# ProgramerSalar/stable-diffusion-from-scratch

Measured on NVIDIA B200. Metric: 512px DDIM-50 images/sec, higher is better.
Workload: dtype bf16

## Files before the change

include/sdb200.h:

```cpp
#ifndef SDB200_H
#define SDB200_H

#include <stdint.h>

#ifdef __cplusplus
extern "C" {
#endif

#define SDB_OK            0
#define SDB_ERR_INVALID  -1
#define SDB_ERR_CUDA     -2
#define SDB_ERR_NOTMA    -3

#define SDB_F32   0
#define SDB_BF16  1

int         sdb_version(void);
const char* sdb_last_error_string(void);
int         sdb_device_sm_count(void);
unsigned long long sdb_launch_count(void);
int sdb_pdl_skip_next(int n);

int sdb_nchw_to_nhwc(const float* src, void* dst, int dst_dtype, int N, int C, int dst_C, int HW, void* stream);
int sdb_nchw_to_nhwc_split(const float* src, void* dst , int N, int C, int dst_C, int HW, void* stream);
// ... 83 lines not shown
    int geglu;
    int col_group, col_group_stride;
    int split_k;
    int block_n;
    int taps;
    int kw;
    int stride, pad_h, pad_w;
    int NB, IH, IW, Cin, OH, OW;
    int cout_pad;
    int out_sh, out_sw, out_oh, out_ow, OHF, OWF;
    void* ws; long long ws_bytes;
    int rows_per_item;
    int variant;
    float* colstats; long long colstats_slots;
    int b_const;
} sdb_tc_args;
int sdb_tc_colstats_layout(const sdb_tc_args* args , long long* slots, long long* slots_per_item);
long long sdb_tc_workspace_bytes(const sdb_tc_args* args );
int sdb_tc_contract(const sdb_tc_args* args , void* stream);
int sdb_tc_set_pair_kernel(int enable);
int sdb_tc_set_tma_epilogue(int enable);
int sdb_tc_set_tail_split(int enable);

typedef struct sdb_attn_args {
    const void* q; const void* k; const void* v; void* out;
    long long q_bs, q_ss, q_hs;
    long long k_bs, k_ss, k_hs;
    long long v_bs, v_ss, v_hs;
    long long o_bs, o_ss, o_hs;
    int B, H, Sq, Sk, d, dpad;
    float scale;
    int dense;
    int causal;
// ... 13 lines not shown
```

stable-diffusion-from-scratch_b200/_lib.py:

```python
import ctypes as C
import os

import torch

HERE = os.path.dirname(os.path.abspath(__file__))
LIB_PATH = os.path.join(HERE, "libsdb200.so")

F32, BF16 = 0, 1

_lib = None


class SdbError(RuntimeError):
    pass


class SimtArgs(C.Structure):
    _fields_ = [
        ("A", C.c_void_p), ("B", C.c_void_p), ("out", C.c_void_p),
        ("bias", C.c_void_p), ("rowvec", C.c_void_p), ("residual", C.c_void_p),
        ("lda", C.c_longlong), ("ldb", C.c_longlong), ("ldc", C.c_longlong), ("ldr", C.c_longlong), ("ldv", C.c_longlong),
        ("M", C.c_int), ("N", C.c_int), ("K", C.c_int),
        ("alpha", C.c_float),
        ("b_kn", C.c_int),
# ... 15 lines not shown
        ("out_dtype", C.c_int),
        ("geglu", C.c_int),
        ("col_group", C.c_int), ("col_group_stride", C.c_int),
        ("split_k", C.c_int),
        ("block_n", C.c_int),
        ("taps", C.c_int), ("kw", C.c_int),
        ("stride", C.c_int), ("pad_h", C.c_int), ("pad_w", C.c_int),
        ("NB", C.c_int), ("IH", C.c_int), ("IW", C.c_int), ("Cin", C.c_int), ("OH", C.c_int), ("OW", C.c_int),
        ("cout_pad", C.c_int),
        ("out_sh", C.c_int), ("out_sw", C.c_int), ("out_oh", C.c_int), ("out_ow", C.c_int), ("OHF", C.c_int), ("OWF", C.c_int),
        ("ws", C.c_void_p), ("ws_bytes", C.c_longlong),
        ("rows_per_item", C.c_int),
        ("variant", C.c_int),
        ("colstats", C.c_void_p), ("colstats_slots", C.c_longlong),
        ("b_const", C.c_int),
    ]


class AttnArgs(C.Structure):
    _fields_ = [
        ("q", C.c_void_p), ("k", C.c_void_p), ("v", C.c_void_p), ("out", C.c_void_p),
        ("q_bs", C.c_longlong), ("q_ss", C.c_longlong), ("q_hs", C.c_longlong),
        ("k_bs", C.c_longlong), ("k_ss", C.c_longlong), ("k_hs", C.c_longlong),
        ("v_bs", C.c_longlong), ("v_ss", C.c_longlong), ("v_hs", C.c_longlong),
        ("o_bs", C.c_longlong), ("o_ss", C.c_longlong), ("o_hs", C.c_longlong),
        ("B", C.c_int), ("H", C.c_int), ("Sq", C.c_int), ("Sk", C.c_int), ("d", C.c_int), ("dpad", C.c_int),
        ("scale", C.c_float),
        ("dense", C.c_int),
        ("causal", C.c_int),
    ]
# ... 29 lines not shown
    "sdb_gather_rows": (_I, [_P, _P, _I, _I, _P, _P]),
    "sdb_skinny_linear": (_I, [_P, _I, _I, _P, _P, _I, _I, _I, _P, _P]),
    "sdb_skinny_linear_bf16w": (_I, [_P, _I, _I, _P, _P, _I, _I, _I, _P, _P]),
    "sdb_ddim_step": (_I, [_P, _P, _P, _F, _P, _F, _F, _F, _F, _F, _F, _P, _P, _L, _P]),
    "sdb_ddim_xprev": (_I, [_P, _P, _P, _F, _P, _F, _F, _F, _F, _P, _L, _P]),
    "sdb_ddpm_step": (_I, [_P, _P, _P, _P, _P, _P, _I, _I, _F, _P, _P, _I, _L, _P]),
    "sdb_inpaint_blend": (_I, [_P, _P, _P, _P, _P, _P, _I, _I, _I, _L, _P, _P]),
    "sdb_diag_gaussian": (_I, [_P, _P, _I, _I, _L, _P, _P, _P, _P, _P, _P]),
    "sdb_q_sample": (_I, [_P, _P, _P, _P, _I, _L, _P, _P]),
    "sdb_simt_contract": (_I, [C.POINTER(SimtArgs), _P]),
    "sdb_tc_contract": (_I, [C.POINTER(TcArgs), _P]),
    "sdb_tc_set_pair_kernel": (_I, [_I]),
    "sdb_tc_set_tma_epilogue": (_I, [_I]),
    "sdb_tc_set_tail_split": (_I, [_I]),
    "sdb_tc_workspace_bytes": (_L, [C.POINTER(TcArgs)]),
    "sdb_tc_colstats_layout": (_I, [C.POINTER(TcArgs), C.POINTER(C.c_longlong), C.POINTER(C.c_longlong)]),
    "sdb_attention_fwd": (_I, [C.POINTER(AttnArgs), _P]),
    "sdb_attention_set_short_key_kernel": (_I, [_I]),
    "sdb_attention_wide_fwd": (_I, [_P, _P, _P, _P, _L, _L, _L, _L, _L, _L, _L, _L, _I, _I, _I, _I, _F, _P]),
}


def load(path=None):
    global _lib
    if _lib is not None and path is None:
        return _lib
    path = path or LIB_PATH
    if not os.path.exists(path):
        raise SdbError(
            "libsdb200.so not found at %s — build it with `python -c 'import __graft_entry__ as g; g.build()'`; "
# ... 51 lines not shown
```

stable-diffusion-from-scratch_b200/csrc/tc_contract.cu:

```cuda
#include "common.cuh"
#include "ptx.cuh"
#include <stdlib.h>
#include <string.h>

namespace sdb {

using namespace ptx;

struct TcP {
    void* out;
    const float* bias; const float* rowvec; const float* residual;
    float* ws; long long ws_split_stride;
    float* colstats; long long colstats_sq;
    long long ldc, ldr, ldv;
    int M, N;
    int kblocks;
    int kpt;
    int out_bf16, geglu;
    int col_group, col_group_stride;
    int split_k;
    int tiles_n;
    int m_pairs;
    int off32;
    int stages;
    int epi_tma;
    int epi_nbuf;
    int epi_bw, epi_bh;
// ... 444 lines not shown
        for (int o = 8; o <= 16; o <<= 1) {
            cs_s.x += __shfl_xor_sync(0xffffffffu, cs_s.x, o); cs_s.y += __shfl_xor_sync(0xffffffffu, cs_s.y, o);
            cs_s.z += __shfl_xor_sync(0xffffffffu, cs_s.z, o); cs_s.w += __shfl_xor_sync(0xffffffffu, cs_s.w, o);
            cs_q.x += __shfl_xor_sync(0xffffffffu, cs_q.x, o); cs_q.y += __shfl_xor_sync(0xffffffffu, cs_q.y, o);
            cs_q.z += __shfl_xor_sync(0xffffffffu, cs_q.z, o); cs_q.w += __shfl_xor_sync(0xffffffffu, cs_q.w, o);
        }
        const int cn = col + 4 * (int)qd;
        if (lane < 8 && cn < n_out) {
            float* dst = p.colstats + (long long)(ub.mt * 4 + lg) * p.N + cn;
            *reinterpret_cast<float4*>(dst) = cs_s;
            *reinterpret_cast<float4*>(dst + p.colstats_sq) = cs_q;
        }
    }
}

template <int BN, int MODE, bool HAS_RES>
__device__ __forceinline__ void epilogue_tma_units(const TcP& p, const CUtensorMap* tmC, const CUtensorMap* tmR, uint32_t tmem_d,
                                                   float* s_bias2, uint32_t stg_a, uint64_t* rbar, uint64_t* tfull_bar,
                                                   uint32_t tempty_leader0, uint32_t tempty_leader1, int warp, int lane, uint32_t rank,
                                                   int pair, int npairs, int units) {
    constexpr bool GEGLU = MODE == EPI_GEGLU;
    constexpr bool OUT16 = MODE != EPI_F32;
    constexpr int COLS = GEGLU ? BN / 2 : BN;
    constexpr int NCHUNK = (COLS + 31) / 32;
    constexpr int CPW_MAX = (NCHUNK + 1) / 2;
    constexpr int ACC_STRIDE = 256;
    const int lg = warp & 3, half = (warp - 4) >> 2;
    const int et = threadIdx.x - 128;
    const int cpw = (NCHUNK - half + 1) / 2;
    const int nbuf = p.epi_nbuf, lead = nbuf - 1;
    const bool partial = p.split_k > 1;
    const float* const biasp = partial ? nullptr : p.bias;
    const float* const rowv = (!partial && p.rowvec && p.conv && MODE == EPI_F32) ? p.rowvec : nullptr;
    const bool want_cs = MODE == EPI_F32 && p.colstats != nullptr && !partial;
    const int n_out = GEGLU ? p.N / 2 : p.N;
// ... 98 lines not shown
                if (lane == 0) mbar_arrive_cluster(buf ? tempty_leader1 : tempty_leader0);
            }
            if (HAS_RES) {
                mbar_wait(rbar + bi, (q / (uint32_t)nbuf) & 1u);
            } else {
                if (lane == 0) tma_store_wait_read<1>();
                __syncwarp();
            }
            tepi_chunk<BN, MODE, HAS_RES>(p, tmC, cur, g, sb_a, sbuf, c0, col, ub, lane, lg, rowmask, img_w, rv_ok, rowv, want_cs, partial, n_out);
            if (HAS_RES) {
                if (lane == 0) tma_store_wait_read<1>();
                issue_residual(q + (uint32_t)lead);
            }
            ++q;
        }
    }
    if (lane == 0) tma_store_wait_read<0>();
    __syncwarp();
}

template <int BN, int MODE, bool HAS_RES>
__device__ __forceinline__ void epilogue_tma_single(const TcP& p, const CUtensorMap* tmC, const CUtensorMap* tmR, uint32_t taddr,
                                                    uint32_t sb_a, uint32_t stg_a, uint64_t* rbar, uint64_t* accum_bar, const UnitBox& ub,
                                                    int lane, int lg, uint32_t rowmask, int img_w, int ncols) {
    constexpr bool GEGLU = MODE == EPI_GEGLU;
    constexpr int COLS = GEGLU ? BN / 2 : BN;
    constexpr int NCHUNK = (COLS + 31) / 32;
    const int nch = ncols >= COLS ? NCHUNK : (ncols + 31) / 32;
    const bool partial = p.split_k > 1;
    const float* const rowv = (!partial && p.rowvec && p.conv && MODE == EPI_F32) ? p.rowvec : nullptr;
// ... 38 lines not shown
tc_contract_kernel(const __grid_constant__ CUtensorMap tmA, const __grid_constant__ CUtensorMap tmB,
                   const __grid_constant__ CUtensorMap tmC, const __grid_constant__ CUtensorMap tmR, const TcP p) {
    pdl_trigger();
    if (threadIdx.x == 0) { TC1_TRACE(0); TC1_TRACE(7); }
    using Cfg = TcCfg<BN>;
    constexpr int STAGES = Cfg::STAGES;
    extern __shared__ uint8_t smem_raw[];
    uint8_t* smem = reinterpret_cast<uint8_t*>((reinterpret_cast<uintptr_t>(smem_raw) + 1023) & ~(uintptr_t)1023);
    uint8_t* sA = smem;
    uint8_t* sB = smem + STAGES * TC_A_BYTES;
    uint64_t* full_bar = reinterpret_cast<uint64_t*>(smem + STAGES * Cfg::STAGE_BYTES);
    uint64_t* empty_bar = full_bar + STAGES;
    uint64_t* accum_bar = empty_bar + STAGES;
    uint32_t* tmem_slot = reinterpret_cast<uint32_t*>(accum_bar + 1);
    uint64_t* res_bar = accum_bar + 2;
    float* s_bias = reinterpret_cast<float*>(smem + STAGES * Cfg::STAGE_BYTES + 256);

    const int warp = threadIdx.x >> 5, lane = threadIdx.x & 31;

    int tile = blockIdx.x;
    int ncols = BN, n_off = 0;
    if (tile >= p.full_tiles) {
        const int t2 = tile - p.full_tiles;
        tile = p.full_tiles + (t2 >> 1);
        if (t2 & 1) { n_off = 96; ncols = BN - 96; } else { ncols = 96; }
    }
    const int nt = tile % p.tiles_n, mt = tile / p.tiles_n;
    const int n0 = nt * BN + n_off;
    const int split = blockIdx.y;
    const int kb0 = (int)((long long)p.kblocks * split / p.split_k);
// ... 119 lines not shown
#define SDB_TEPI1(MODE, RES) epilogue_tma_single<BN, MODE, RES>(p, &tmC, &tmR, taddr, smem_u32(s_bias), stg_a, rbar, accum_bar, ub, lane, lg, rowmask, img_w, ncols)
            if (p.geglu) {
                if constexpr (BN % 64 == 0) SDB_TEPI1(EPI_GEGLU, false);
            } else if (p.split_k > 1) SDB_TEPI1(EPI_F32, false);
            else if (p.out_bf16) SDB_TEPI1(EPI_BF16, false);
            else if (p.residual != nullptr) SDB_TEPI1(EPI_F32, true);
            else SDB_TEPI1(EPI_F32, false);
#undef SDB_TEPI1
        } else {
            prefetch_residual_row(p, pix, n0, BN);
            float* stage = reinterpret_cast<float*>(sA) + (warp - 2) * (EPI_WARP_BYTES / 4);
            if (warp == 2 && lane == 0) TC1_TRACE(4);
            epilogue_warp<BN>(p, taddr, s_bias, stage, lane, n0, nt, pix, img, split, 0, 1, accum_bar, 0, mt * 4 + lg, ncols);
            if (warp == 2 && lane == 0) TC1_TRACE(5);
        }
    }

    tcgen05_fence_before();
    __syncthreads();
    if (warp == 1) {
        tcgen05_fence_after();
        tmem_dealloc(tmem_d, Cfg::TMEM_COLS);
    }
}

constexpr int TC2_MAX_STAGES = 8;
constexpr int TC2_SMEM_LIMIT = 232448;

template <int BN, int EW>
struct Tc2Cfg {
// ... 16 lines not shown
                        const __grid_constant__ CUtensorMap tmC, const __grid_constant__ CUtensorMap tmR, const TcP p) {
    pdl_trigger();
    using Cfg = Tc2Cfg<BN, EW>;
    constexpr int TC2_EPI_WARPS = EW;
    const int STAGES = p.stages;
    extern __shared__ uint8_t smem_raw[];
    uint8_t* smem = reinterpret_cast<uint8_t*>((reinterpret_cast<uintptr_t>(smem_raw) + 1023) & ~(uintptr_t)1023);
    uint8_t* sA = smem;
    uint8_t* sB = smem + STAGES * TC_A_BYTES;
    uint64_t* full_bar = reinterpret_cast<uint64_t*>(smem + STAGES * Cfg::STAGE_BYTES);
    uint64_t* empty_bar = full_bar + TC2_MAX_STAGES;
    uint64_t* tfull_bar = empty_bar + TC2_MAX_STAGES;
    uint64_t* tempty_bar = tfull_bar + 2;
    uint32_t* tmem_slot = reinterpret_cast<uint32_t*>(tempty_bar + 2);
    uint64_t* res_bar = tempty_bar + 4;
    float* s_bias = reinterpret_cast<float*>(smem + STAGES * Cfg::STAGE_BYTES + 512);
    uint8_t* staging = reinterpret_cast<uint8_t*>((reinterpret_cast<uintptr_t>(s_bias + 2 * BN) + 1023) & ~(uintptr_t)1023);

    const int warp = threadIdx.x >> 5, lane = threadIdx.x & 31;
    const uint32_t rank = cluster_ctarank();
    const int pair = blockIdx.x >> 1, npairs = gridDim.x >> 1;
    const int units = p.m_pairs * p.tiles_n * p.split_k;

    if (warp == 0 && lane == 0) {
        tma_prefetch_desc(&tmA);
        tma_prefetch_desc(&tmB);
        for (int s = 0; s < STAGES; ++s) { mbar_init(&full_bar[s], 1); mbar_init(&empty_bar[s], 1); }
        for (int b = 0; b < 2; ++b) { mbar_init(&tfull_bar[b], 1); mbar_init(&tempty_bar[b], 2 * TC2_EPI_WARPS); }
        for (int b = 0; b < 3 * EW && EW == 8; ++b) mbar_init(&res_bar[b], 1);
        fence_barrier_init();
// ... 71 lines not shown
                    const uint64_t bdesc = bdesc0 + (uint64_t)(s * (Cfg::B_HALF_BYTES >> 4));
#pragma unroll
                    for (int k = 0; k < TC_BK / 16; ++k)
                        umma_bf16_ss_pair(acc, adesc + 2 * k, bdesc + 2 * k, idesc, (kb > kb0 || k > 0) ? 1u : 0u);
                    umma_commit_pair(&empty_bar[s], 3);
                    if (++s == STAGES) { s = 0; ph ^= 1; }
                }
                umma_commit_pair(&tfull_bar[buf], 3);
                TC_TRACE(2, it);
            }
        }
    } else if (warp >= 4 && EW == 8 && p.epi_tma) {
        const uint32_t tl0 = mapa_u32(&tempty_bar[0], 0), tl1 = mapa_u32(&tempty_bar[1], 0);
        const uint32_t stg_a = smem_u32(staging) + (uint32_t)(warp - 4) * (uint32_t)(p.epi_nbuf * TEPI_BOX_BYTES);
        uint64_t* rbar = res_bar + 3 * (warp - 4);
#define SDB_TEPI(MODE, RES) epilogue_tma_units<BN, MODE, RES>(p, &tmC, &tmR, tmem_d, s_bias, stg_a, rbar, tfull_bar, tl0, tl1, warp, lane, rank, pair, npairs, units)
        if (p.geglu) {
            if constexpr (BN % 64 == 0) SDB_TEPI(EPI_GEGLU, false);
        } else if (p.split_k > 1) SDB_TEPI(EPI_F32, false);
        else if (p.out_bf16) SDB_TEPI(EPI_BF16, false);
        else if (p.residual != nullptr) SDB_TEPI(EPI_F32, true);
        else SDB_TEPI(EPI_F32, false);
#undef SDB_TEPI
    } else if (warp >= 4) {
        const int et = threadIdx.x - 128;
        const int lg = warp & 3;
        const int half = (warp - 4) >> 2;
        const int row = lg * 32 + lane;
        const uint32_t tempty_leader0 = mapa_u32(&tempty_bar[0], 0);
        const uint32_t tempty_leader1 = mapa_u32(&tempty_bar[1], 0);
        float* stage = reinterpret_cast<float*>(staging) + (warp - 4) * (EPI_WARP_BYTES / 4);
        auto row_of = [&](int mt, int& img) -> long long {
            img = 0;
            if (p.conv) {
// ... 29 lines not shown
            for (int i = et; i < BN; i += 32 * TC2_EPI_WARPS) {
                int n = n0 + i;
                s_bias[i] = (p.bias && n < p.N) ? p.bias[n] : 0.f;
            }
            named_bar_sync(1, 32 * TC2_EPI_WARPS);
            int img = 0;
            const long long pix = row_of(mt, img);
            const uint32_t taddr = tmem_d + ((uint32_t)(lg * 32) << 16) + buf * Cfg::ACC_STRIDE;
            if (warp == 4 && lane == 0) TC_TRACE(3, it);
            epilogue_warp<BN>(p, taddr, s_bias, stage, lane, n0, nt, pix, img, split, half, EW / 4, &tfull_bar[buf], (it >> 1) & 1,
                              mt * 4 + lg);
            if (warp == 4 && lane == 0) TC_TRACE(4, it);
            tcgen05_fence_before();
            __syncwarp();
            if (lane == 0) mbar_arrive_cluster(buf ? tempty_leader1 : tempty_leader0);
        }
    }

    __syncwarp();
    tcgen05_fence_before();
    cluster_sync_all();
    if (warp == 2) {
        tcgen05_fence_after();
        tmem_dealloc_pair(tmem_d, 512);
    }
}

typedef CUresult (*PFN_encodeTiled)(CUtensorMap*, CUtensorMapDataType, cuuint32_t, void*, const cuuint64_t*,
                                    const cuuint64_t*, const cuuint32_t*, const cuuint32_t*, CUtensorMapInterleave,
                                    CUtensorMapSwizzle, CUtensorMapL2promotion, CUtensorMapFloatOOBfill);
// ... 384 lines not shown
}

extern "C" int sdb_tc_colstats_layout(const sdb_tc_args* a, long long* slots, long long* slots_per_item) {
    if (!a || !slots || !slots_per_item) return SDB_ERR_INVALID;
    *slots = 0; *slots_per_item = 0;
    sdb_tc_args t = *a;
    if (t.split_k == 0 && !t.ws) t.ws = reinterpret_cast<void*>(16);
    TcPlan pl;
    int rc = make_plan(&t, &pl);
    if (rc) return rc;
    if (!colstats_supported(a, pl)) return SDB_OK;
    colstats_layout(a, pl, slots, slots_per_item);
    return SDB_OK;
}

extern "C" int sdb_tc_contract(const sdb_tc_args* a, void* stream) {
    SDB_REQUIRE(a && a->A && a->B && a->out, "tc_contract: null pointer");
    TcPlan pl;
    int rc = make_plan(a, &pl);
    if (rc) return rc;
    if (a->colstats) {
        SDB_REQUIRE(colstats_supported(a, pl), "tc_contract: column statistics need an fp32 conv output whose 32-row slots lie inside one sample");
        long long need_slots = 0, spi_ = 0;
        colstats_layout(a, pl, &need_slots, &spi_);
        SDB_REQUIRE(a->colstats_slots >= need_slots, "tc_contract: colstats buffer has %lld slots, needs %lld", a->colstats_slots, need_slots);
        SDB_REQUIRE(((uintptr_t)a->colstats & 15) == 0 && ((uintptr_t)a->out & 15) == 0 && (!a->residual || (((uintptr_t)a->residual & 15) == 0 && a->ldr % 4 == 0)) &&
                    (!a->rowvec || (((uintptr_t)a->rowvec & 15) == 0 && a->ldv % 4 == 0)), "tc_contract: column statistics need 16-byte aligned operands");
    }
    const bool conv = a->taps > 0;
    const int bn = pl.bn;
// ... 12 lines not shown
    p.col_group = a->col_group; p.col_group_stride = a->col_group_stride;
    p.split_k = pl.split_k;
    if (p.split_k > 1) {
        SDB_REQUIRE(a->ws && a->ws_bytes >= pl.ws_bytes, "tc_contract: split_k=%d needs a %lld-byte workspace (got %lld)",
                    p.split_k, pl.ws_bytes, a->ws ? a->ws_bytes : 0LL);
        SDB_REQUIRE(((uintptr_t)a->ws & 15) == 0, "tc_contract: workspace must be 16-byte aligned");
        p.ws = reinterpret_cast<float*>(a->ws);
        p.ws_split_stride = pl.rows_out * a->N;
    }
    {
        const long long ld_max = a->ldc > a->N ? a->ldc : a->N;
        p.off32 = (pl.rows_out + 1) * ld_max + a->N < (1LL << 32) ? 1 : 0;
    }
    p.colstats = pl.split_k > 1 ? nullptr : a->colstats;
    p.colstats_sq = a->colstats ? a->colstats_slots * (long long)a->N : 0;
#ifdef SDB_TC_TRACE
    p.trace = g_trace_ptr;
#endif
    p.tiles_n = pl.tiles_n;
    p.conv = conv;
    p.cout_pad = conv ? a->cout_pad : 0;

    CUtensorMap tmA, tmB;
    const int m_tiles = pl.m_tiles;
    const int taps = pl.taps;
    if (conv) {
        p.tw = pl.tw; p.th = pl.th; p.tn = pl.tn;
        p.kw = a->kw; p.stride = a->stride; p.pad_h = a->pad_h; p.pad_w = a->pad_w;
        p.NB = a->NB; p.OH = a->OH; p.OW = a->OW;
        p.tiles_w = pl.tiles_w; p.tiles_h = pl.tiles_h;
// ... 81 lines not shown
    if (use_pair) {
        switch (bn) {
            case 128: rc = launch_tc_pair<128>(tmA, tmB, tmC, tmR, p, m_tiles, st); break;
            case 160: rc = launch_tc_pair<160>(tmA, tmB, tmC, tmR, p, m_tiles, st); break;
            default: rc = launch_tc_pair<256>(tmA, tmB, tmC, tmR, p, m_tiles, st); break;
        }
    } else {
        switch (bn) {
            case 32: rc = launch_tc<32>(tmA, tmB, tmC, tmR, p, m_tiles, st); break;
            case 64: rc = launch_tc<64>(tmA, tmB, tmC, tmR, p, m_tiles, st); break;
            case 128: rc = launch_tc<128>(tmA, tmB, tmC, tmR, p, m_tiles, st); break;
            case 160: rc = launch_tc<160>(tmA, tmB, tmC, tmR, p, m_tiles, st); break;
            default: rc = launch_tc<256>(tmA, tmB, tmC, tmR, p, m_tiles, st); break;
        }
    }
    if (rc || p.split_k == 1) return rc;
    ReduceRemap rm;
    memset(&rm, 0, sizeof(rm));
    long long red_rows = pl.rows_out;
    if (conv && (p.out_sh != 1 || p.out_sw != 1 || p.out_oh != 0 || p.out_ow != 0 || p.OHF != p.OH || p.OWF != p.OW)) {
        rm.on = 1; rm.OH = p.OH; rm.OW = p.OW; rm.sh = p.out_sh; rm.sw = p.out_sw; rm.oh0 = p.out_oh; rm.ow0 = p.out_ow;
        rm.OHF = p.OHF; rm.OWF = p.OWF;
        red_rows = (long long)p.NB * p.OH * p.OW;
    }
    const long long total = red_rows * (a->N / 4);
    int blocks = (int)((total + 255) / 256);
    if (blocks > 148 * 8) blocks = 148 * 8;
    const long long rows_per_img = conv ? (long long)p.OHF * p.OWF : 1;
    if (a->colstats) {
        SDB_REQUIRE(!p.out_bf16 && ((uintptr_t)a->out & 15) == 0 && a->ldc % 4 == 0 && (!a->bias || ((uintptr_t)a->bias & 15) == 0),
                    "tc_contract: split-K column statistics need 16-byte aligned fp32 operands");
        dim3 g((unsigned)(pl.rows_out / 32), (unsigned)((a->N / 4 + 31) / 32));
        launch_pdl(splitk_reduce_stats_kernel, dim3(g), dim3(256), 0, st, p.ws, p.ws_split_stride, p.split_k, pl.rows_out, a->N, a->bias,
                   conv ? a->rowvec : nullptr, a->ldv, rows_per_img, a->residual, a->ldr, reinterpret_cast<float*>(a->out), a->ldc,
                   a->colstats, p.colstats_sq);
        return check_launch("splitk_reduce_stats_kernel");
    }
    launch_pdl(splitk_reduce_kernel, dim3(blocks), dim3(256), 0, st, p.ws, p.ws_split_stride, p.split_k, red_rows, a->N, a->bias,
                                                 conv ? a->rowvec : nullptr, a->ldv, rows_per_img, a->residual, a->ldr,
                                                 a->out, a->ldc, p.out_bf16, rm);
    return check_launch("splitk_reduce_kernel");
}
```

stable-diffusion-from-scratch_b200/ops.py:

```python
import ctypes as C
import os

import torch

from . import _lib
from ._lib import BF16, F32, AttnArgs, SimtArgs, TcArgs, check, dtype_code, ptr, require_cuda, stream_ptr


def _L():
    return _lib.load()


def nchw_to_nhwc(x, out_dtype=torch.float32, pad_to=0, split=False, x1=None):
    require_cuda(x, x1)
    assert x.dtype == torch.float32 and x.is_contiguous()
    N, Cc, H, W = x.shape
    C1 = 0
    if x1 is not None:
        assert x1.dtype == torch.float32 and x1.is_contiguous() and x1.dim() == 4
        assert x1.shape[0] == N and tuple(x1.shape[2:]) == (H, W), "nchw_to_nhwc: x1 %s does not match x %s" % (
            tuple(x1.shape), tuple(x.shape))
        C1 = x1.shape[1]
    Ct = Cc + C1
    Cd = max(Ct, pad_to)
# ... 11 lines not shown


def nhwc_to_nchw(x):
    require_cuda(x)
    assert x.dtype == torch.float32 and x.is_contiguous()
    N, H, W, Cc = x.shape
    out = torch.empty((N, Cc, H, W), dtype=torch.float32, device=x.device)
    check(_L().sdb_nhwc_to_nchw(ptr(x), ptr(out), N, Cc, H * W, stream_ptr()), "nhwc_to_nchw")
    return out


_gn_counters = {}
_USE_COLSTATS = os.environ.get("SDB200_COLSTATS", "1") != "0"


def _gn_ticket_buffer(dev, n):
    key = (dev.index, torch.cuda.current_stream(dev).cuda_stream)
    buf = _gn_counters.get(key)
    if buf is None or buf.numel() < n:
        buf = torch.zeros(max(n, 1024), dtype=torch.int32, device=dev)
        _gn_counters[key] = buf
    return buf


def groupnorm(x0, gamma, beta, eps, act=0, out_dtype=torch.float32, x1=None, groups=32, exact=False, want_raw=False):
    require_cuda(x0, x1, gamma, beta)
    assert x0.dtype == torch.float32 and x0.is_contiguous()
    N, H, W, C0 = x0.shape
    gbs = 0
    if gamma.dim() == 2:
        assert gamma.shape == beta.shape and gamma.shape[0] == N and gamma.stride(1) == 1 and beta.stride() == gamma.stride()
        gbs = gamma.stride(0)
    C1 = 0
    if x1 is not None:
        assert x1.dtype == torch.float32 and x1.is_contiguous() and x1.shape[:3] == x0.shape[:3]
        C1 = x1.shape[3]
    Ct = C0 + C1
# ... 358 lines not shown
    if a.split_k or a.variant or (a.block_n and not a.geglu):
        return
    if _PLANS is None:
        _PLANS = _plan_table()
    key = (kind, int(rows_per_sample), a.N, a.K, a.taps, a.stride if a.taps else 0, a.geglu, int(bool(a.residual)),
           a.out_dtype, a.col_group)
    hit = _PLANS.get(key)
    if hit is not None:
        if a.geglu:
            if hit[1] == a.block_n:
                a.variant = hit[0]
        else:
            a.variant, a.block_n, a.split_k = hit[0], hit[1], hit[2]


def _tc_launch(a, what):
    lib = _L()
    need = lib.sdb_tc_workspace_bytes(C.byref(a))
    if need < 0:
        check(-1, what)
    ws = None
    if need > 0:
        ws = torch.empty(need, dtype=torch.uint8, device=torch.device("cuda", torch.cuda.current_device()))
        a.ws, a.ws_bytes = ws.data_ptr(), need
    check(lib.sdb_tc_contract(C.byref(a), stream_ptr()), what)


def conv_tc(x, w_rskc, bias, kh, kw, stride=1, pad=0, rowvec=None, residual=None, out_dtype=torch.float32,
            split_k=0, block_n=0, out=None, phase=None, variant=0, want_stats=False, stats_into=None, pad_hi=None, b_const=False):
    require_cuda(x, w_rskc, bias, rowvec, residual, out)
    assert x.dtype == torch.bfloat16 and w_rskc.dtype == torch.bfloat16 and x.is_contiguous() and w_rskc.is_contiguous()
    N, IH, IW, Cin = x.shape
    taps, Cout, Cin2 = w_rskc.shape
    assert Cin2 == Cin and taps == kh * kw
    a = TcArgs()
    if phase is None:
        pad_hi = pad if pad_hi is None else pad_hi
        OH = (IH + pad + pad_hi - kh) // stride + 1
        OW = (IW + pad + pad_hi - kw) // stride + 1
        pad_h = pad_w = pad
        if out is None:
            out = torch.empty((N, OH, OW, Cout), dtype=out_dtype, device=x.device)
        a.out_sh = a.out_sw = 1
        a.out_oh = a.out_ow = 0
# ... 19 lines not shown
    a.NB, a.IH, a.IW, a.Cin, a.OH, a.OW = N, IH, IW, Cin, OH, OW
    a.cout_pad = Cout
    a.b_const = int(bool(b_const))
    if residual is not None:
        assert residual.dtype == torch.float32 and residual.is_contiguous()
    _apply_plan(a, "conv", OH * OW)
    cs = None
    if stats_into is not None:
        cs_t, total_slots, first_slot = stats_into
        a.colstats, a.colstats_slots = cs_t.data_ptr() + 4 * first_slot * Cout, total_slots
    elif want_stats and phase is None and out.dtype == torch.float32:
        slots, spi = tc_colstats_layout(a)
        if slots > 0:
            cs = torch.empty((2, slots, Cout), dtype=torch.float32, device=x.device)
            a.colstats, a.colstats_slots = cs.data_ptr(), slots
    _tc_launch(a, "tc conv")
    if cs is not None:
        out._sdb_cs = (cs, slots, spi, 1, 0)
    return out


def tc_colstats_layout(a):
    slots, spi = C.c_longlong(0), C.c_longlong(0)
    check(_L().sdb_tc_colstats_layout(C.byref(a), C.byref(slots), C.byref(spi)), "tc colstats layout")
    return slots.value, spi.value


UP2_PHASES = ((0, 0), (0, 1), (1, 0), (1, 1))


def fold_upsample_weights(w, dtype):
# ... 39 lines not shown
    N, IH, IW, Cin = x.shape
    taps, Cout, _ = w_rskc.shape
    sh, sw, o_h, o_w, OHF, OWF, pad_h, pad_w = phase
    a.out_sh, a.out_sw, a.out_oh, a.out_ow, a.OHF, a.OWF = sh, sw, o_h, o_w, OHF, OWF
    a.A, a.B, a.out = ptr(x), ptr(w_rskc), ptr(out)
    a.bias = ptr(bias)
    a.lda, a.ldb, a.ldc, a.ldr = Cin, Cin, Cout, Cout
    a.M, a.N, a.K = N * IH * IW, Cout, taps * Cin
    a.out_dtype = dtype_code(out.dtype)
    a.taps, a.kw, a.stride, a.pad_h, a.pad_w = taps, kw, stride, pad_h, pad_w
    a.NB, a.IH, a.IW, a.Cin, a.OH, a.OW = N, IH, IW, Cin, IH, IW
    a.cout_pad = Cout


def gemm_tc(A, W, bias=None, residual=None, out_dtype=torch.float32, geglu=False, col_group=0, col_group_stride=0,
            split_k=0, block_n=0, out=None, ldc=None, M=None, lda=None, rows_per_item=0, variant=0, b_const=False):
    require_cuda(A, W, bias, residual, out)
    assert A.dtype == torch.bfloat16 and W.dtype == torch.bfloat16 and W.is_contiguous()
    K = A.shape[-1]
    if M is None:
        M = A.numel() // K
    N = W.shape[0]
    assert W.shape[1] == K
    n_out = N // 2 if geglu else N
    if out is None:
        width = (N // col_group) * col_group_stride if col_group else n_out
        if col_group:
            out = torch.zeros((M, width), dtype=out_dtype, device=A.device)
        else:
            out = torch.empty((M, width), dtype=out_dtype, device=A.device)
    a = TcArgs()
# ... 4 lines not shown
    a.ldc = ldc if ldc is not None else out.stride(-2)
    a.ldr = residual.stride(-2) if residual is not None else 0
    a.ldv = 0
    a.M, a.N, a.K = M, N, K
    a.out_dtype = dtype_code(out.dtype)
    a.geglu = int(bool(geglu))
    a.col_group, a.col_group_stride = col_group, col_group_stride
    a.split_k = split_k
    a.block_n = block_n
    a.variant = variant
    a.taps = 0
    a.rows_per_item = int(rows_per_item)
    a.b_const = int(bool(b_const))
    if rows_per_item:
        _apply_plan(a, "gemm", rows_per_item)
    _tc_launch(a, "tc gemm")
    return out


def attention_tc(q, k, v, B, H, Sq, Sk, d, dpad, scale, q_strides, k_strides, v_strides, out=None, o_strides=None, dense=False,
                 causal=False):
    require_cuda(q, k, v)
    assert q.dtype == k.dtype == v.dtype == torch.bfloat16
    if out is None:
        out = torch.empty((B, Sq, H * d), dtype=torch.bfloat16, device=q.device)
    a = AttnArgs()
    a.q, a.k, a.v, a.out = ptr(q), ptr(k), ptr(v), ptr(out)
    a.q_bs, a.q_ss, a.q_hs = q_strides
    a.k_bs, a.k_ss, a.k_hs = k_strides
    a.v_bs, a.v_ss, a.v_hs = v_strides
    a.o_bs, a.o_ss, a.o_hs = o_strides if o_strides is not None else (Sq * H * d, H * d, d)
# ... 17 lines not shown
```

Measured before the change: 14.90.

## Fuse split-K reduction into GEMM epilogue via last-arrival ticket fix-up

Split-K partial tiles are now reduced inside the tensor-core kernel. The last CTA to arrive on a per-tile atomic ticket sums all partials from the workspace and applies bias, rowvec, residual and optional column statistics. This removes the separate split-K reduce (and stats) kernel launch and its dependency gap. In exchange it adds threadfences, atomics and a serialized fix-up on one CTA per tile, plus a persistent ticket buffer that must be reset to zero.

```diff
diff --git a/include/sdb200.h b/include/sdb200.h
--- a/include/sdb200.h
+++ b/include/sdb200.h
@@ -121,9 +121,11 @@
     int variant;
     float* colstats; long long colstats_slots;
     int b_const;
+    int* splitk_tickets; long long splitk_tickets_len;
 } sdb_tc_args;
 int sdb_tc_colstats_layout(const sdb_tc_args* args , long long* slots, long long* slots_per_item);
 long long sdb_tc_workspace_bytes(const sdb_tc_args* args );
+long long sdb_tc_splitk_tickets(const sdb_tc_args* args );
 int sdb_tc_contract(const sdb_tc_args* args , void* stream);
 int sdb_tc_set_pair_kernel(int enable);
 int sdb_tc_set_tma_epilogue(int enable);
diff --git a/stable-diffusion-from-scratch_b200/_lib.py b/stable-diffusion-from-scratch_b200/_lib.py
--- a/stable-diffusion-from-scratch_b200/_lib.py
+++ b/stable-diffusion-from-scratch_b200/_lib.py
@@ -53,6 +53,7 @@
         ("variant", C.c_int),
         ("colstats", C.c_void_p), ("colstats_slots", C.c_longlong),
         ("b_const", C.c_int),
+        ("splitk_tickets", C.c_void_p), ("splitk_tickets_len", C.c_longlong),
     ]
 
 
@@ -112,6 +113,7 @@
     "sdb_tc_set_tma_epilogue": (_I, [_I]),
     "sdb_tc_set_tail_split": (_I, [_I]),
     "sdb_tc_workspace_bytes": (_L, [C.POINTER(TcArgs)]),
+    "sdb_tc_splitk_tickets": (_L, [C.POINTER(TcArgs)]),
     "sdb_tc_colstats_layout": (_I, [C.POINTER(TcArgs), C.POINTER(C.c_longlong), C.POINTER(C.c_longlong)]),
     "sdb_attention_fwd": (_I, [C.POINTER(AttnArgs), _P]),
     "sdb_attention_set_short_key_kernel": (_I, [_I]),
diff --git a/stable-diffusion-from-scratch_b200/csrc/tc_contract.cu b/stable-diffusion-from-scratch_b200/csrc/tc_contract.cu
--- a/stable-diffusion-from-scratch_b200/csrc/tc_contract.cu
+++ b/stable-diffusion-from-scratch_b200/csrc/tc_contract.cu
@@ -11,6 +11,8 @@
     void* out;
     const float* bias; const float* rowvec; const float* residual;
     float* ws; long long ws_split_stride;
+    int* tickets;
+    int fix_stats;
     float* colstats; long long colstats_sq;
     long long ldc, ldr, ldv;
     int M, N;
@@ -485,11 +487,199 @@
     }
 }
 
-template <int BN, int MODE, bool HAS_RES>
+
+__device__ __forceinline__ long long tile_row_pix(const TcP& p, int mt, int r, int& img) {
+    img = 0;
+    if (!p.conv) return (long long)mt * TC_BM + r < p.M ? (long long)mt * TC_BM + r : -1;
+    const int tww = mt % p.tiles_w, thh = (mt / p.tiles_w) % p.tiles_h, tnb = mt / (p.tiles_w * p.tiles_h);
+    const int in_ = r / (p.th * p.tw), rem = r - in_ * (p.th * p.tw);
+    const int ih = rem / p.tw, iw = rem - ih * p.tw;
+    img = tnb * p.tn + in_;
+    const int oh = thh * p.th + ih, ow = tww * p.tw + iw;
+    if (img >= p.NB || oh >= p.OH || ow >= p.OW) return -1;
+    return ((long long)img * p.OHF + (oh * p.out_sh + p.out_oh)) * p.OWF + (ow * p.out_sw + p.out_ow);
+}
+
+__device__ __forceinline__ bool splitk_last_arrival(const TcP& p, int tile, bool tma_stored, int lane, bool leader, int nthreads,
+                                                    volatile int* s_flag) {
+    if (tma_stored) {
+        if (lane == 0) {
+            tma_store_wait_all<0>();
+            asm volatile("fence.proxy.async.global;" ::: "memory");
+        }
+        __syncwarp();
+    }
+    __threadfence();
+    named_bar_sync(2, nthreads);
+    if (leader) {
+        const int last = atomicAdd(p.tickets + tile, 1) == p.split_k - 1;
+        if (last) p.tickets[tile] = 0;
+        *s_flag = last;
+    }
+    named_bar_sync(2, nthreads);
+    const bool last = *s_flag != 0;
+    if (last) __threadfence();
+    return last;
+}
+
+template <int BN>
+__device__ __noinline__ void splitk_fixup(const TcP p, int mt, int n0, int tid, int nthreads, int wid, int nwarps, int lane) {
+    const int ncols = p.N - n0 < BN ? p.N - n0 : BN;
+    const int nq = ncols >> 2;
+    const float* const rowv = p.conv ? p.rowvec : nullptr;
+    const long long rows_per_img = p.conv ? (long long)p.OHF * p.OWF : 1;
+    const float4 z4 = make_float4(0.f, 0.f, 0.f, 0.f);
+    auto ld4s = [](const float* q) { return make_float4(q[0], q[1], q[2], q[3]); };
+    auto add4 = [](float4& a, const float4& b) { a.x += b.x; a.y += b.y; a.z += b.z; a.w += b.w; };
+    if (!p.fix_stats) {
+        constexpr int UNR = 4;
+        const int items = TC_BM * nq;
+        for (int i0 = tid; i0 < items; i0 += UNR * nthreads) {
+            float4 acc[UNR], q1[UNR], bv[UNR], rv[UNR], re[UNR];
+            long long m[UNR];
+            int n[UNR];
+#pragma unroll
+            for (int j = 0; j < UNR; ++j) {
+                const int i = i0 + j * nthreads;
+                const int r = i / nq;
+                int img;
+                m[j] = i < items ? tile_row_pix(p, mt, r, img) : -1;
+                n[j] = n0 + 4 * (i - r * nq);
+                const bool ok = m[j] >= 0;
+                const float* src = p.ws + m[j] * p.N + n[j];
+                acc[j] = ok ? __ldcg(reinterpret_cast<const float4*>(src)) : z4;
+                q1[j] = ok ? __ldcg(reinterpret_cast<const float4*>(src + p.ws_split_stride)) : z4;
+                bv[j] = ok && p.bias ? ld4s(p.bias + n[j]) : z4;
+                rv[j] = ok && rowv ? ld4s(rowv + (m[j] / rows_per_img) * p.ldv + n[j]) : z4;
+                re[j] = ok && p.residual ? ld4s(p.residual + m[j] * p.ldr + n[j]) : z4;
+            }
+#pragma unroll
+            for (int j = 0; j < UNR; ++j) add4(acc[j], q1[j]);
+            for (int s = 2; s < p.split_k; s += 2) {
+                const bool two = s + 1 < p.split_k;
+                float4 v0[UNR], v1[UNR];
+#pragma unroll
+                for (int j = 0; j < UNR; ++j) {
+                    const float* src = p.ws + s * p.ws_split_stride + m[j] * p.N + n[j];
+                    v0[j] = m[j] >= 0 ? __ldcg(reinterpret_cast<const float4*>(src)) : z4;
+                    v1[j] = m[j] >= 0 && two ? __ldcg(reinterpret_cast<const float4*>(src + p.ws_split_stride)) : z4;
+                }
+#pragma unroll
+                for (int j = 0; j < UNR; ++j) {
+                    add4(acc[j], v0[j]);
+                    if (two) add4(acc[j], v1[j]);
+                }
+            }
+#pragma unroll
+            for (int j = 0; j < UNR; ++j) {
+                if (m[j] < 0) continue;
+                float4 a = acc[j];
+                if (p.bias) add4(a, bv[j]);
+                if (rowv) add4(a, rv[j]);
+                if (p.residual) add4(a, re[j]);
+                if (p.out_bf16) {
+                    __nv_bfloat16* o = reinterpret_cast<__nv_bfloat16*>(p.out) + m[j] * p.ldc + n[j];
+                    o[0] = __float2bfloat16_rn(a.x); o[1] = __float2bfloat16_rn(a.y);
+                    o[2] = __float2bfloat16_rn(a.z); o[3] = __float2bfloat16_rn(a.w);
+                } else {
+                    float* o = reinterpret_cast<float*>(p.out) + m[j] * p.ldc + n[j];
+                    o[0] = a.x; o[1] = a.y; o[2] = a.z; o[3] = a.w;
+                }
+            }
+        }
+        return;
+    }
+    const int rg = lane >> 2, qi = lane & 3;
+    const int qgroups = (nq + 3) >> 2;
+    const int witems = 4 * qgroups;
+    for (int w0 = wid; w0 < witems; w0 += 2 * nwarps) {
+        float4 acc[2][4], q1[2][4], re[2][4], b4[2], rv[2];
+        long long m0[2];
+        int n[2];
+        bool ok[2];
+#pragma unroll
+        for (int u = 0; u < 2; ++u) {
+            const int w = w0 + u * nwarps;
+            const int q = w / qgroups, quad = 4 * (w - q * qgroups) + qi;
+            int img;
+            m0[u] = w < witems ? tile_row_pix(p, mt, 32 * q, img) : -1;
+            n[u] = n0 + 4 * quad;
+            ok[u] = m0[u] >= 0 && quad < nq;
+            b4[u] = ok[u] && p.bias ? __ldg(reinterpret_cast<const float4*>(p.bias + n[u])) : z4;
+            rv[u] = ok[u] && rowv ? __ldg(reinterpret_cast<const float4*>(rowv + (m0[u] / rows_per_img) * p.ldv + n[u])) : z4;
+#pragma unroll
+            for (int r = 0; r < 4; ++r) {
+                const long long mm = m0[u] + 4 * rg + r;
+                const float* src = p.ws + mm * p.N + n[u];
+                acc[u][r] = ok[u] ? __ldcg(reinterpret_cast<const float4*>(src)) : z4;
+                q1[u][r] = ok[u] ? __ldcg(reinterpret_cast<const float4*>(src + p.ws_split_stride)) : z4;
+                re[u][r] = ok[u] && p.residual ? __ldg(reinterpret_cast<const float4*>(p.residual + mm * p.ldr + n[u])) : z4;
+            }
+        }
+#pragma unroll
+        for (int u = 0; u < 2; ++u)
+#pragma unroll
+            for (int r = 0; r < 4; ++r) add4(acc[u][r], q1[u][r]);
+        for (int s = 2; s < p.split_k; s += 2) {
+            const bool two = s + 1 < p.split_k;
+            float4 v0[2][4], v1[2][4];
+#pragma unroll
+            for (int u = 0; u < 2; ++u)
+#pragma unroll
+                for (int r = 0; r < 4; ++r) {
+                    const float* src = p.ws + s * p.ws_split_stride + (m0[u] + 4 * rg + r) * p.N + n[u];
+                    v0[u][r] = ok[u] ? __ldcg(reinterpret_cast<const float4*>(src)) : z4;
+                    v1[u][r] = ok[u] && two ? __ldcg(reinterpret_cast<const float4*>(src + p.ws_split_stride)) : z4;
+                }
+#pragma unroll
+            for (int u = 0; u < 2; ++u)
+#pragma unroll
+                for (int r = 0; r < 4; ++r) {
+                    add4(acc[u][r], v0[u][r]);
+                    if (two) add4(acc[u][r], v1[u][r]);
+                }
+        }
+#pragma unroll
+        for (int u = 0; u < 2; ++u) {
+            if (m0[u] < 0) continue;
+            float4 cs = z4, cq = z4;
+            if (ok[u]) {
+#pragma unroll
+                for (int r = 0; r < 4; ++r) {
+                    float4 a = acc[u][r];
+                    add4(a, b4[u]);
+                    if (rowv) add4(a, rv[u]);
+                    if (p.residual) add4(a, re[u][r]);
+                    *reinterpret_cast<float4*>(reinterpret_cast<float*>(p.out) + (m0[u] + 4 * rg + r) * p.ldc + n[u]) = a;
+                    add4(cs, a);
+                    cq.x = fmaf(a.x, a.x, cq.x); cq.y = fmaf(a.y, a.y, cq.y); cq.z = fmaf(a.z, a.z, cq.z); cq.w = fmaf(a.w, a.w, cq.w);
+                }
+            }
+            float4 ts = cs, tq = cq;
+#pragma unroll
+            for (int g = 1; g < 8; ++g) {
+                const int src = 4 * g + qi;
+                const float4 vs = make_float4(__shfl_sync(0xffffffffu, cs.x, src), __shfl_sync(0xffffffffu, cs.y, src),
+                                              __shfl_sync(0xffffffffu, cs.z, src), __shfl_sync(0xffffffffu, cs.w, src));
+                const float4 vq = make_float4(__shfl_sync(0xffffffffu, cq.x, src), __shfl_sync(0xffffffffu, cq.y, src),
+                                              __shfl_sync(0xffffffffu, cq.z, src), __shfl_sync(0xffffffffu, cq.w, src));
+                add4(ts, vs);
+                add4(tq, vq);
+            }
+            if (rg == 0 && ok[u]) {
+                float* dst = p.colstats + (m0[u] >> 5) * p.N + n[u];
+                *reinterpret_cast<float4*>(dst) = ts;
+                *reinterpret_cast<float4*>(dst + p.colstats_sq) = tq;
+            }
+        }
+    }
+}
+
+template <int BN, int MODE, bool HAS_RES, bool FIXUP = false>
 __device__ __forceinline__ void epilogue_tma_units(const TcP& p, const CUtensorMap* tmC, const CUtensorMap* tmR, uint32_t tmem_d,
                                                    float* s_bias2, uint32_t stg_a, uint64_t* rbar, uint64_t* tfull_bar,
                                                    uint32_t tempty_leader0, uint32_t tempty_leader1, int warp, int lane, uint32_t rank,
-                                                   int pair, int npairs, int units) {
+                                                   int pair, int npairs, int units, volatile int* s_flag) {
     constexpr bool GEGLU = MODE == EPI_GEGLU;
     constexpr bool OUT16 = MODE != EPI_F32;
     constexpr int COLS = GEGLU ? BN / 2 : BN;
@@ -618,6 +808,8 @@
             }
             ++q;
         }
+        if (FIXUP && splitk_last_arrival(p, ub.mt * p.tiles_n + ub.nt, true, lane, et == 0, 32 * 8, s_flag))
+            splitk_fixup<BN>(p, ub.mt, ub.nt * BN, et, 32 * 8, warp - 4, 8, lane);
     }
     if (lane == 0) tma_store_wait_read<0>();
     __syncwarp();
@@ -686,6 +878,7 @@
     uint64_t* accum_bar = empty_bar + STAGES;
     uint32_t* tmem_slot = reinterpret_cast<uint32_t*>(accum_bar + 1);
     uint64_t* res_bar = accum_bar + 2;
+    volatile int* s_flag = reinterpret_cast<volatile int*>(res_bar + 4);
     float* s_bias = reinterpret_cast<float*>(smem + STAGES * Cfg::STAGE_BYTES + 256);
 
     const int warp = threadIdx.x >> 5, lane = threadIdx.x & 31;
@@ -835,6 +1028,8 @@
             epilogue_warp<BN>(p, taddr, s_bias, stage, lane, n0, nt, pix, img, split, 0, 1, accum_bar, 0, mt * 4 + lg, ncols);
             if (warp == 2 && lane == 0) TC1_TRACE(5);
         }
+        if (p.tickets != nullptr && splitk_last_arrival(p, tile, p.epi_tma != 0, lane, et == 0, 128, s_flag))
+            splitk_fixup<BN>(p, mt, n0, et, 128, warp - 2, 4, lane);
     }
 
     tcgen05_fence_before();
@@ -881,6 +1076,7 @@
     uint64_t* tempty_bar = tfull_bar + 2;
     uint32_t* tmem_slot = reinterpret_cast<uint32_t*>(tempty_bar + 2);
     uint64_t* res_bar = tempty_bar + 4;
+    volatile int* s_flag = reinterpret_cast<volatile int*>(res_bar + 3 * EW);
     float* s_bias = reinterpret_cast<float*>(smem + STAGES * Cfg::STAGE_BYTES + 512);
     uint8_t* staging = reinterpret_cast<uint8_t*>((reinterpret_cast<uintptr_t>(s_bias + 2 * BN) + 1023) & ~(uintptr_t)1023);
 
@@ -982,10 +1178,13 @@
         const uint32_t tl0 = mapa_u32(&tempty_bar[0], 0), tl1 = mapa_u32(&tempty_bar[1], 0);
         const uint32_t stg_a = smem_u32(staging) + (uint32_t)(warp - 4) * (uint32_t)(p.epi_nbuf * TEPI_BOX_BYTES);
         uint64_t* rbar = res_bar + 3 * (warp - 4);
-#define SDB_TEPI(MODE, RES) epilogue_tma_units<BN, MODE, RES>(p, &tmC, &tmR, tmem_d, s_bias, stg_a, rbar, tfull_bar, tl0, tl1, warp, lane, rank, pair, npairs, units)
+#define SDB_TEPI(MODE, RES, ...) epilogue_tma_units<BN, MODE, RES, ##__VA_ARGS__>(p, &tmC, &tmR, tmem_d, s_bias, stg_a, rbar, tfull_bar, tl0, tl1, warp, lane, rank, pair, npairs, units, s_flag)
         if (p.geglu) {
             if constexpr (BN % 64 == 0) SDB_TEPI(EPI_GEGLU, false);
-        } else if (p.split_k > 1) SDB_TEPI(EPI_F32, false);
+        } else if (p.split_k > 1) {
+            if (p.tickets != nullptr) SDB_TEPI(EPI_F32, false, true);
+            else SDB_TEPI(EPI_F32, false);
+        }
         else if (p.out_bf16) SDB_TEPI(EPI_BF16, false);
         else if (p.residual != nullptr) SDB_TEPI(EPI_F32, true);
         else SDB_TEPI(EPI_F32, false);
@@ -1045,6 +1244,8 @@
             tcgen05_fence_before();
             __syncwarp();
             if (lane == 0) mbar_arrive_cluster(buf ? tempty_leader1 : tempty_leader0);
+            if (p.tickets != nullptr && splitk_last_arrival(p, mt * p.tiles_n + nt, false, lane, et == 0, 32 * TC2_EPI_WARPS, s_flag))
+                splitk_fixup<BN>(p, mt, n0, et, 32 * TC2_EPI_WARPS, warp - 4, TC2_EPI_WARPS, lane);
         }
     }
 
@@ -1459,6 +1660,22 @@
     return SDB_OK;
 }
 
+static long long splitk_fixup_tickets(const sdb_tc_args* a, const TcPlan& pl) {
+    if (pl.split_k <= 1) return 0;
+    if (a->colstats && !(a->taps > 0 && pl.tw == a->OW && (pl.tn == 1 || pl.th == a->OH))) return 0;
+    const long long mt = pl.use_pair ? 2LL * ((pl.m_tiles + 1) / 2) : pl.m_tiles;
+    return mt * pl.tiles_n;
+}
+
+extern "C" long long sdb_tc_splitk_tickets(const sdb_tc_args* a) {
+    if (!a) return -1;
+    sdb_tc_args t = *a;
+    if (t.split_k == 0 && !t.ws) t.ws = reinterpret_cast<void*>(16);
+    TcPlan pl;
+    if (make_plan(&t, &pl) != SDB_OK) return -1;
+    return splitk_fixup_tickets(&t, pl);
+}
+
 extern "C" int sdb_tc_contract(const sdb_tc_args* a, void* stream) {
     SDB_REQUIRE(a && a->A && a->B && a->out, "tc_contract: null pointer");
     TcPlan pl;
@@ -1501,6 +1718,17 @@
     }
     p.colstats = pl.split_k > 1 ? nullptr : a->colstats;
     p.colstats_sq = a->colstats ? a->colstats_slots * (long long)a->N : 0;
+    const long long tickets = a->splitk_tickets ? splitk_fixup_tickets(a, pl) : 0;
+    if (tickets > 0) {
+        SDB_REQUIRE(a->splitk_tickets_len >= tickets, "tc_contract: split-K fix-up needs %lld tickets (got %lld)", tickets, a->splitk_tickets_len);
+        SDB_REQUIRE(((uintptr_t)a->splitk_tickets & 3) == 0, "tc_contract: split-K tickets must be 4-byte aligned");
+        p.tickets = a->splitk_tickets;
+        p.fix_stats = a->colstats != nullptr;
+        p.colstats = a->colstats;
+    }
+    if (pl.split_k > 1 && a->colstats)
+        SDB_REQUIRE(!p.out_bf16 && ((uintptr_t)a->out & 15) == 0 && a->ldc % 4 == 0 && (!a->bias || ((uintptr_t)a->bias & 15) == 0),
+                    "tc_contract: split-K column statistics need 16-byte aligned fp32 operands");
 #ifdef SDB_TC_TRACE
     p.trace = g_trace_ptr;
 #endif
@@ -1612,7 +1840,7 @@
             default: rc = launch_tc<256>(tmA, tmB, tmC, tmR, p, m_tiles, st); break;
         }
     }
-    if (rc || p.split_k == 1) return rc;
+    if (rc || p.split_k == 1 || p.tickets) return rc;
     ReduceRemap rm;
     memset(&rm, 0, sizeof(rm));
     long long red_rows = pl.rows_out;
@@ -1626,8 +1854,6 @@
     if (blocks > 148 * 8) blocks = 148 * 8;
     const long long rows_per_img = conv ? (long long)p.OHF * p.OWF : 1;
     if (a->colstats) {
-        SDB_REQUIRE(!p.out_bf16 && ((uintptr_t)a->out & 15) == 0 && a->ldc % 4 == 0 && (!a->bias || ((uintptr_t)a->bias & 15) == 0),
-                    "tc_contract: split-K column statistics need 16-byte aligned fp32 operands");
         dim3 g((unsigned)(pl.rows_out / 32), (unsigned)((a->N / 4 + 31) / 32));
         launch_pdl(splitk_reduce_stats_kernel, dim3(g), dim3(256), 0, st, p.ws, p.ws_split_stride, p.split_k, pl.rows_out, a->N, a->bias,
                    conv ? a->rowvec : nullptr, a->ldv, rows_per_img, a->residual, a->ldr, reinterpret_cast<float*>(a->out), a->ldc,
diff --git a/stable-diffusion-from-scratch_b200/ops.py b/stable-diffusion-from-scratch_b200/ops.py
--- a/stable-diffusion-from-scratch_b200/ops.py
+++ b/stable-diffusion-from-scratch_b200/ops.py
@@ -49,13 +49,20 @@
 _USE_COLSTATS = os.environ.get("SDB200_COLSTATS", "1") != "0"
 
 
-def _gn_ticket_buffer(dev, n):
+_tc_counters = {}
+
+
+def _ticket_buffer(pool, dev, n):
     key = (dev.index, torch.cuda.current_stream(dev).cuda_stream)
-    buf = _gn_counters.get(key)
+    buf = pool.get(key)
     if buf is None or buf.numel() < n:
         buf = torch.zeros(max(n, 1024), dtype=torch.int32, device=dev)
-        _gn_counters[key] = buf
+        pool[key] = buf
     return buf
+
+
+def _gn_ticket_buffer(dev, n):
+    return _ticket_buffer(_gn_counters, dev, n)
 
 
 def groupnorm(x0, gamma, beta, eps, act=0, out_dtype=torch.float32, x1=None, groups=32, exact=False, want_raw=False):
@@ -444,20 +451,29 @@
             a.variant, a.block_n, a.split_k = hit[0], hit[1], hit[2]
 
 
-def _tc_launch(a, what):
+def _tc_launch(a, what, splitk_fixup=True):
     lib = _L()
     need = lib.sdb_tc_workspace_bytes(C.byref(a))
     if need < 0:
         check(-1, what)
     ws = None
     if need > 0:
-        ws = torch.empty(need, dtype=torch.uint8, device=torch.device("cuda", torch.cuda.current_device()))
+        dev = torch.device("cuda", torch.cuda.current_device())
+        ws = torch.empty(need, dtype=torch.uint8, device=dev)
         a.ws, a.ws_bytes = ws.data_ptr(), need
+        if splitk_fixup:
+            nt = lib.sdb_tc_splitk_tickets(C.byref(a))
+            if nt < 0:
+                check(-1, what)
+            if nt > 0:
+                t = _ticket_buffer(_tc_counters, dev, nt)
+                a.splitk_tickets, a.splitk_tickets_len = t.data_ptr(), t.numel()
     check(lib.sdb_tc_contract(C.byref(a), stream_ptr()), what)
 
 
 def conv_tc(x, w_rskc, bias, kh, kw, stride=1, pad=0, rowvec=None, residual=None, out_dtype=torch.float32,
-            split_k=0, block_n=0, out=None, phase=None, variant=0, want_stats=False, stats_into=None, pad_hi=None, b_const=False):
+            split_k=0, block_n=0, out=None, phase=None, variant=0, want_stats=False, stats_into=None, pad_hi=None, b_const=False,
+            splitk_fixup=True):
     require_cuda(x, w_rskc, bias, rowvec, residual, out)
     assert x.dtype == torch.bfloat16 and w_rskc.dtype == torch.bfloat16 and x.is_contiguous() and w_rskc.is_contiguous()
     N, IH, IW, Cin = x.shape
@@ -507,7 +523,7 @@
         if slots > 0:
             cs = torch.empty((2, slots, Cout), dtype=torch.float32, device=x.device)
             a.colstats, a.colstats_slots = cs.data_ptr(), slots
-    _tc_launch(a, "tc conv")
+    _tc_launch(a, "tc conv", splitk_fixup)
     if cs is not None:
         out._sdb_cs = (cs, slots, spi, 1, 0)
     return out
@@ -577,7 +593,8 @@
 
 
 def gemm_tc(A, W, bias=None, residual=None, out_dtype=torch.float32, geglu=False, col_group=0, col_group_stride=0,
-            split_k=0, block_n=0, out=None, ldc=None, M=None, lda=None, rows_per_item=0, variant=0, b_const=False):
+            split_k=0, block_n=0, out=None, ldc=None, M=None, lda=None, rows_per_item=0, variant=0, b_const=False,
+            splitk_fixup=True):
     require_cuda(A, W, bias, residual, out)
     assert A.dtype == torch.bfloat16 and W.dtype == torch.bfloat16 and W.is_contiguous()
     K = A.shape[-1]
@@ -612,7 +629,7 @@
     a.b_const = int(bool(b_const))
     if rows_per_item:
         _apply_plan(a, "gemm", rows_per_item)
-    _tc_launch(a, "tc gemm")
+    _tc_launch(a, "tc gemm", splitk_fixup)
     return out
 
 
```

Result: slower. 13.39, median of 6 (-10.1%).
